# uiuc-robovision/video-dqn

Hardware: AMD Instinct MI355X
Metric: (s,a,r,s') TD-updates/sec, 224x224 frames, batch 256, 1/2/4/8 MI355X (higher is better)
Workload: dtype bf16; 1 GPU; HabitatDQNMultiAction ResNet-18 extra_capacity, 5 categories x 3 actions, full TD update (online fwd on [s;s'], target fwd on s', Double-DQN target + L2 TD loss, backward, Adam); batch_per_gpu=256, global_batch=256, frame=224x224x3 uint8 (normalise fused), parallelism=dp1, target_update_interval=1000, loss_clip=rect, loss_kind=l2, minibatch_pool=4, frame_pack=at the start of every update

## Files before the change

video_dqn_amd/csrc/engine.hip:

```cpp
#include "engine_net.h"

bool wgrad_two_stage() {
  static const bool on = [] { const char* e = getenv("VDQN_WGRAD_TWO_STAGE"); return e && e[0] == '1'; }();
  return on;
}

namespace {

bool side_ready(vdqn_net* net) {
  if (!net->overlap) return false;
  if (!net->side) {
    int prio = 0;
    {
      const char* e = getenv("VDQN_SIDE_PRIORITY");
      int lo = 0, hi = 0;
      if (hipDeviceGetStreamPriorityRange(&lo, &hi) == hipSuccess) prio = (!e || e[0] == 'l') ? lo : (e[0] == 'h' ? hi : 0);
    }
    if (hipStreamCreateWithPriority(&net->side, hipStreamNonBlocking, prio) != hipSuccess ||
        hipStreamCreateWithPriority(&net->side2, hipStreamNonBlocking, prio) != hipSuccess) {
      net->overlap = 0;
      net->side = nullptr;
      net->side2 = nullptr;
      return false;
    }
// ... 533 lines not shown
  }
  RC(run_dgrad(net, c1, pk, bw + W.g_h[b], gx, n, resid, x, st));
  return VDQN_OK;
}

}

extern "C" int vdqn_net_backward_begin(vdqn_net* net, const vdqn_step_args* a, const float* dq_f32, void* stream) {
  VDQN_CHECK(net && a && dq_f32, "vdqn_net_backward_begin: null arg");
  VDQN_CHECK(!net->basic(), "vdqn_net_backward_begin: only extra_capacity (eval-mode BatchNorm) has a per-call backward; ARCHITECTURE='basic' trains through vdqn_net_td_forward");
  VDQN_CHECK(a->params && a->bnstats && a->packed_online && a->acts_online && a->bwd && a->grads, "vdqn_net_backward_begin: null buffer");
  VDQN_CHECK(a->batch >= 1 && a->batch <= net->cfg.max_batch && a->acts_samples == a->batch,
             "vdqn_net_backward_begin: acts_samples (%d) must equal batch (%d) <= max_batch", a->acts_samples, a->batch);
  hipStream_t st = (hipStream_t)stream;
  const int B = a->batch;
  const BwdLayout W = bwd_layout(net, B);
  unsigned char* bw = (unsigned char*)a->bwd;
  hipError_t e = hipMemsetAsync(bw + W.zero_begin, 0, (size_t)W.zero_bytes, st);
  VDQN_CHECK(e == hipSuccess, "vdqn_net_backward_begin: memset failed: %s", hipGetErrorString(e));
  launch_dq_pad(net, dq_f32, bw + W.dq, B, st);
  VDQN_LAUNCH_CHECK();
  return VDQN_OK;
}

extern "C" void* vdqn_net_grad_stream(vdqn_net* net) {
  if (!net || !side_ready(net)) return nullptr;
  return (void*)net->side;
}

extern "C" int vdqn_net_backward_stage(vdqn_net* net, const vdqn_step_args* a, int32_t stage, void* stream) {
  VDQN_CHECK(net && a && a->grads, "vdqn_net_backward_stage: null arg");
  VDQN_CHECK(stage >= 0 && stage < 3, "vdqn_net_backward_stage: stage %d", stage);
  hipStream_t st = (hipStream_t)stream;
  const int B = a->batch, F = net->cfg.num_frames, n = B * F, dt = net->cfg.dtype;
  const bool gtb = a->train_on_ground_truth != 0;
  const ActLayout A = act_layout(net, step_layout_samples(net, a));
  const BwdLayout W = bwd_layout(net, B);
  const unsigned char* pk = (const unsigned char*)a->packed_online;
  unsigned char* ao = (unsigned char*)a->acts_online;
  unsigned char* bw = (unsigned char*)a->bwd;
  bool split_conv1 = false;
  int part_rows[kMaxLayers];
  std::fill(part_rows, part_rows + kMaxLayers, kTileRows);

  if (net->basic()) {
    if (stage == 0) {
      const Layer& top = net->layers[net->l_top4];
      RC(run_wgrad(net, top, bw, W, bw + W.dq, ao + A.avg, B, wgrad_stream(net, st), true));
      RC(run_dgrad(net, top, pk, bw + W.dq, bw + W.g_avg, B, nullptr, nullptr, st));
      RC(vdqn_avgpool_bwd(bw + W.g_avg, ao + A.o[7], bw + W.g_o[7], n, 49, 512, dt, st));
      RC(block_backward_train(net, a, 7, A, W, n, st));
      RC(block_backward_train(net, a, 6, A, W, n, st));
    } else if (stage == 1) {
      RC(block_backward_train(net, a, 5, A, W, n, st));
      RC(block_backward_train(net, a, 4, A, W, n, st));
    } else {
      for (int b = 3; b >= 0; --b) RC(block_backward_train(net, a, b, A, W, n, st));
      RC(vdqn_maxpool_bwd(bw + W.g_pool, ao + A.idx, nullptr, bw + W.g_c1, n, 112, 112, 64, dt, st));
      RC(run_bn_bwd(net, a, net->l_conv1, A, bw + W.g_c1, ao + A.r_c1, bw + W.g_c1, n, st));
      RC(run_wgrad(net, net->layers[net->l_conv1], bw, W, bw + W.g_c1, a->packed_frames ? a->packed_frames : ao + A.t_in, n, wgrad_stream(net, st)));
    }
  } else if (stage == 0) {
    const Layer& t4 = net->layers[net->l_top4];
    const Layer& t2 = net->layers[net->l_top2];
    const Layer& t0 = net->layers[net->l_top0];
    const Layer& f8 = net->layers[net->l_f8];
    RC(run_wgrad(net, t4, bw, W, bw + W.dq, ao + A.l1, B, wgrad_stream(net, st), true));
    RC(run_dgrad(net, t4, pk, bw + W.dq, bw + W.g_l1, B, nullptr, ao + A.l1, st, bw + W.part[kPartL1], nullptr, nullptr, &part_rows[net->l_top2]));
    RC(run_wgrad(net, t2, bw, W, bw + W.g_l1, ao + A.l0, B, wgrad_stream(net, st)));
    RC(run_dgrad(net, t2, pk, bw + W.g_l1, bw + W.g_l0, B, nullptr, ao + A.l0, st, bw + W.part[kPartL0], nullptr, nullptr, &part_rows[net->l_top0]));
    RC(run_wgrad(net, t0, bw, W, bw + W.g_l0, ao + A.f8, B, wgrad_stream(net, st)));
    RC(run_dgrad(net, t0, pk, bw + W.g_l0, bw + W.g_f8, B, nullptr, ao + A.f8, st, bw + W.part[kPartF8], nullptr, nullptr, &part_rows[net->l_f8]));
    RC(run_wgrad(net, f8, bw, W, bw + W.g_f8, ao + A.o[7], n, wgrad_stream(net, st)));
    RC(run_dgrad(net, f8, pk, bw + W.g_f8, bw + W.g_o[7], n, nullptr, ao + A.o[7], st, bw + W.part[part_o(7)]));
    RC(block_backward(net, a, 7, A, W, n, st));
    RC(block_backward(net, a, 6, A, W, n, st));
  } else if (stage == 1) {
    RC(block_backward(net, a, 5, A, W, n, st));
    RC(block_backward(net, a, 4, A, W, n, st));
  } else {
    for (int b = 3; b >= 0; --b) RC(block_backward(net, a, b, A, W, n, st));
    split_conv1 = net->overlap && net->side && net->l_conv1 == net->layer_stage_first[2] && net->layer_stage_count[2] > 1;
  }
  int max_co = 0;
  for (int i = net->layer_stage_first[stage]; i < net->layer_stage_first[stage] + net->layer_stage_count[stage]; ++i)
    max_co = net->layers[i].co > max_co ? net->layers[i].co : max_co;
  PartTable pt;
  memset(&pt, 0, sizeof(pt));
  for (int i = net->layer_stage_first[stage]; i < net->layer_stage_first[stage] + net->layer_stage_count[stage]; ++i) {
    const int buf = part_buf(net, i);
    if (buf < 0) continue;
    const PartInfo pi = part_info(net, buf, B, part_rows[i]);
    VDQN_CHECK(pi.entries <= pi.capacity, "vdqn_net_backward_stage: layer %s has %d column-sum entries, its buffer holds %lld",
               net->layers[i].name.c_str(), pi.entries, (long long)pi.capacity);
    pt.off[i] = W.part[buf]; pt.tiles[i] = pi.entries; pt.ld[i] = pi.ld; pt.groups[i] = pi.groups; pt.gstride[i] = pi.gstride;
  }
  const bool stem_tail = stage == 2 && !net->basic();
  auto conv1_chain = [&]() -> int {
    const Layer& L1 = net->layers[net->l_conv1];
    static const bool fuse_pool = [] { const char* e = getenv("VDQN_FUSE_POOL_BWD"); return !(e && e[0] == '0'); }();
    const int64_t det_need = net->cfg.deterministic ? vdqn_stem_wgrad_pool_workspace_bytes(n) : 0;
    if (fuse_pool && dt == VDQN_BF16 && (int64_t)n * 115 * 115 * 32 < (1ll << 31) && det_need <= W.det_ws_bytes) {
      prof_layer(L1, n);
      static const bool on_main_env = [] { const char* e = getenv("VDQN_STEM_WGRAD_MAIN"); return !(e && e[0] == '0'); }();
      const bool on_main = g_stem_wgrad_main_override >= 0 ? g_stem_wgrad_main_override != 0 : on_main_env;
      const bool main_st = on_main && split_conv1 && !net->cfg.deterministic;
      return vdqn_stem_wgrad_pool(bw + W.g_pool, ao + A.idx, a->packed_frames ? a->packed_frames : ao + A.t_in, reinterpret_cast<float*>(bw + L1.dw_off), n,
                                  net->cfg.deterministic ? bw + W.det_ws : nullptr, W.det_ws_bytes, main_st ? st : fork(net, st));
    }
    RC(vdqn_maxpool_bwd(bw + W.g_pool, ao + A.idx, nullptr, bw + W.g_c1, n, 112, 112, 64, dt, st));
    RC(run_wgrad(net, L1, bw, W, bw + W.g_c1, a->packed_frames ? a->packed_frames : ao + A.t_in, n, wgrad_stream(net, st)));
    return VDQN_OK;
  };
  if (stem_tail && !split_conv1) RC(conv1_chain());
  hipStream_t us = fork(net, st);
  if (wgrad_two_streams(net)) join(net, net->side2, net->side);
  const double unfold_bytes = (double)(net->stage_end[stage] - net->stage_begin[stage]) * 12.0;
  const int first = net->layer_stage_first[stage], count = net->layer_stage_count[stage];
  if (split_conv1) {
    launch_unfold(net, pt, first + 1, count - 1, max_co, 0, a, us, unfold_bytes);
    RC(conv1_chain());
    if (wgrad_two_streams(net)) join(net, net->side2, net->side);
    (void)fork(net, st);
    launch_unfold(net, pt, net->l_conv1, 1, net->layers[net->l_conv1].co, 0, a, net->side, 0.0);
  } else {
    launch_unfold(net, pt, first, count, max_co, net->basic() ? 1 : 0, a, us, unfold_bytes);
  }
  if (stage == 2) join(net, net->side, st);
  VDQN_LAUNCH_CHECK();
  return VDQN_OK;
}
```

video_dqn_amd/csrc/engine_net.h:

```cpp
#pragma once
#include <math.h>
#include <stdarg.h>
#include <stdlib.h>

#include <algorithm>
#include <string>
#include <vector>

#include "common.h"

#pragma GCC visibility push(hidden)

constexpr int kMaxLayers = 24;
constexpr float kBnEps = 1e-5f;
constexpr float kBnMomentum = 0.1f;

enum LayerKind { K_CONV = 0, K_CONV1_S2D = 1, K_LINEAR = 2, K_LINEAR_PERM = 3 };

struct Layer {
  std::string name, bn_name;
  int kind;
  int co, ci, r, s, stride, pad;
  int has_bn, has_bias;
  int k_ci, k_r, k_s, pix_stride;
// ... 16 lines not shown
  int tile_begin;
};
struct FoldTable {
  int n, n_tiles;
  FoldDesc d[kMaxLayers];
};
struct PartTable {
  int64_t off[kMaxLayers];
  int tiles[kMaxLayers], ld[kMaxLayers], groups[kMaxLayers], gstride[kMaxLayers];
};

enum PartBuf { kPartL1 = 0, kPartL0, kPartF8, kPartPool, kPartBlocks, kPartBufs = kPartBlocks + 16 };
inline int part_o(int b) { return kPartBlocks + 2 * b; }
inline int part_h(int b) { return kPartBlocks + 2 * b + 1; }
constexpr int kTileRows = 128;
struct PartInfo {
  int entries, ld, groups, gstride;
  int64_t capacity;
};

struct ActLayout {
  int64_t t_in, c1, pool, idx;
  int64_t h[8], o[8], ds[8];
  int64_t f8, l0, l1, q, qf;
  int64_t avg, r_c1, r_h[8], r_o[8], r_ds[8], bnw[kMaxLayers], bnw_begin, bnw_bytes, bn_sync;
  int64_t bn_det = -1, bn_det_bytes = 0;
  int64_t total;
};
struct BwdLayout {
  int64_t zero_begin, zero_bytes;
  int64_t dq, g_l1, g_l0, g_f8, g_o[8], g_h[8], dsg[8], g_pool, g_c1;
  int64_t part[kPartBufs];
  int64_t g_avg, g_or[8], g_dsr[8];
  int64_t det_ws, det_ws_bytes;
  int64_t total;
};

inline int64_t align_up(int64_t v, int64_t a = 256) { return (v + a - 1) / a * a; }

#pragma GCC visibility pop

struct vdqn_net {
  vdqn_net_config cfg;
  int gemm_dtype;
  int esz;
  std::vector<Layer> layers;
  std::vector<vdqn_param_info> params;
  int64_t trainable_numel, params_numel, bnstats_numel, packed_bytes;
  int64_t stage_begin[3], stage_end[3];
  int layer_stage_first[3], layer_stage_count[3];
  int64_t dw_bytes;
  FoldTable fold;
  int l_conv1, l_f8, l_top0, l_top2, l_top4;
  bool basic() const { return cfg.extra_capacity == 0; }
  int l_b_conv1[8], l_b_conv2[8], l_b_ds[8];
  BnSync bn_sync = {nullptr, nullptr, nullptr, 1};
  int wgrad_rr = 0;
  int overlap = 1;
  hipStream_t side = nullptr;
  hipStream_t side2 = nullptr;
  std::vector<hipEvent_t> events;
  size_t ev_next = 0;
};

#pragma GCC visibility push(hidden)

#define RC(x)                     \
  do {                            \
    int rc_ = (x);                \
    if (rc_ != VDQN_OK) return rc_; \
  } while (0)

inline int64_t frame_bytes(const vdqn_net* net) { return (int64_t)115 * 115 * 16 * net->esz; }
inline int block_planes(int b) { return 64 << (b / 2); }
inline int block_side(int b) { return 56 >> (b / 2); }

ActLayout act_layout(const vdqn_net* net, int n_samples);
BwdLayout bwd_layout(const vdqn_net* net, int n_samples);
vdqn_wgrad_args wgrad_shape_args(const vdqn_net* net, const Layer& L, int n_units);
int64_t wgrad_max_imgs(const vdqn_net* net, const Layer& L);
int part_buf(const vdqn_net* net, int li);
PartInfo part_info(const vdqn_net* net, int buf, int n_samples, int rows_per_entry);
bool wgrad_two_stage();
void launch_unfold(const vdqn_net* net, const PartTable& pt, int first_layer, int n_layers, int max_co, int raw, const vdqn_step_args* a,
                   hipStream_t stream, double bytes);
void launch_dq_pad(const vdqn_net* net, const float* dq_f32, void* dst, int rows, hipStream_t stream);

#pragma GCC visibility pop
```

video_dqn_amd/csrc/fold.hip:

```cpp
#include "engine_net.h"

namespace {

__device__ __forceinline__ long fold_src_index(const FoldDesc& d, int co, int k) {
  if (d.kind == K_CONV1_S2D) {
    const int a = k >> 6, j = (k >> 4) & 3, ch = k & 15;
    if (ch >= 12) return -1;
    const int bh = ch / 6, bw = (ch / 3) & 1, c = ch % 3;
    const int r7 = 2 * a + bh - 1, s7 = 2 * j + bw - 1;
    if (r7 < 0 || s7 < 0) return -1;
    return ((long)(co * 3 + c) * 7 + r7) * 7 + s7;
  } else if (d.kind == K_LINEAR_PERM) {
    const int f = k / 1600, rem = k - f * 1600;
    const int hw = rem >> 6, c = rem & 63;
    return (long)co * d.ci + f * 1600 + c * 25 + hw;
  } else {
    const int tap = k / d.k_ci, c = k - tap * d.k_ci;
    const int kr = tap / d.k_s, ks = tap - kr * d.k_s;
    return (((long)co * d.ci + c) * d.r + kr) * d.s + ks;
  }
}

__device__ __forceinline__ float fold_scale(const FoldDesc& d, const float* params, const float* bnstats, int co, int raw) {
  if (!d.has_bn || raw) return 1.0f;
  return params[d.g_off + co] / sqrtf(bnstats[d.var_off + co] + kBnEps);
}

template <typename T>
__global__ __launch_bounds__(256) void fold_kernel(const FoldTable tab, const float* __restrict__ params, const float* __restrict__ bnstats,
                                                   unsigned char* __restrict__ packed, int with_dgrad, int raw, int first_layer) {
  const FoldDesc& d = tab.d[first_layer + blockIdx.y];
  const int which = blockIdx.z;
  if (d.tiled) return;
  if (which == 1 && (!with_dgrad || d.wd_off < 0)) return;
  const long stride = (long)gridDim.x * blockDim.x;
  if (which == 0) {
    T* wf = reinterpret_cast<T*>(packed + d.wf_off);
    float* bias = reinterpret_cast<float*>(packed + d.bias_off);
    float* scale = reinterpret_cast<float*>(packed + d.scale_off);
    const long total = (long)d.co_pad * d.kf;
    for (long i = (long)blockIdx.x * blockDim.x + threadIdx.x; i < total; i += stride) {
      const int row = (int)(i / d.kf), k = (int)(i - (long)row * d.kf);
      float v = 0.f;
      if (row < d.co) {
        const float sc = fold_scale(d, params, bnstats, row, raw);
        const long src = fold_src_index(d, row, k);
        if (src >= 0) v = params[d.w_off + src] * sc;
        if (k == 0) {
          scale[row] = sc;
          float b = 0.f;
          if (d.has_bn) b = raw ? 0.f : params[d.b_off + row] - bnstats[d.mean_off + row] * sc;
          else if (d.has_bias) b = params[d.b_off + row];
          bias[row] = b;
        }
      } else if (k == 0) {
        scale[row] = 0.f;
        bias[row] = 0.f;
      }
      wf[i] = from_f32<T>(v);
    }
  } else {
    T* wd = reinterpret_cast<T*>(packed + d.wd_off);
    const long total = (long)d.cd_rows * d.kd;
    for (long i = (long)blockIdx.x * blockDim.x + threadIdx.x; i < total; i += stride) {
      const int n = (int)(i / d.kd), kk = (int)(i - (long)n * d.kd);
      const int tap = kk / d.co_pad, co = kk - tap * d.co_pad;
      float v = 0.f;
      if (co < d.co) {
        const long src = fold_src_index(d, co, tap * d.k_ci + n);
        if (src >= 0) v = params[d.w_off + src] * fold_scale(d, params, bnstats, co, raw);
      }
      wd[i] = from_f32<T>(v);
    }
  }
}

#ifndef VDQN_FOLD_COT
#define VDQN_FOLD_COT 32
#endif
constexpr int kFoldCot = VDQN_FOLD_COT;

template <typename T, int TAPS>
__device__ __forceinline__ void fold_tile_body(const FoldDesc& d, const float* __restrict__ params, const float* __restrict__ bnstats,
                                               unsigned char* __restrict__ packed, int with_dgrad, int raw, float* sW, float* s_scale, int t, int cot_sub) {
  constexpr int COT = kFoldCot;
  constexpr int RUN = 64 * TAPS;
  constexpr int PITCH = RUN + 1;
  const int ci_tiles = d.ci / 64;
  const int cot = t / ci_tiles, cit = t - cot * ci_tiles;
  const int co0 = cot * 64 + cot_sub * COT, c0 = cit * 64;
  if (threadIdx.x < COT) {
    const int co = co0 + threadIdx.x;
    const float sc = co < d.co ? fold_scale(d, params, bnstats, co, raw) : 0.f;
    s_scale[threadIdx.x] = sc;
    if (cit == 0) {
      float b = 0.f;
      if (co < d.co) {
        if (d.has_bn) b = raw ? 0.f : params[d.b_off + co] - bnstats[d.mean_off + co] * sc;
        else if (d.has_bias) b = params[d.b_off + co];
      }
      reinterpret_cast<float*>(packed + d.bias_off)[co] = b;
      reinterpret_cast<float*>(packed + d.scale_off)[co] = sc;
    }
  }
  __syncthreads();
#pragma unroll 6
  for (int i = threadIdx.x; i < COT * RUN / 4; i += 256) {
    const int co_l = i / (RUN / 4), q = i - co_l * (RUN / 4);
    const int co = co0 + co_l;
    float4 v = make_float4(0.f, 0.f, 0.f, 0.f);
    if (co < d.co) v = *reinterpret_cast<const float4*>(params + d.w_off + ((long)co * d.ci + c0) * TAPS + 4 * q);
    const float sc = s_scale[co_l];
    float* dst = sW + co_l * PITCH + 4 * q;
    dst[0] = v.x * sc; dst[1] = v.y * sc; dst[2] = v.z * sc; dst[3] = v.w * sc;
  }
  __syncthreads();
  T* wf = reinterpret_cast<T*>(packed + d.wf_off);
  constexpr int V16 = (int)(8 * sizeof(T) / 16);
#pragma unroll 3
  for (int i = threadIdx.x; i < COT * TAPS * 8; i += 256) {
    const int co_l = i / (TAPS * 8), rem = i - co_l * (TAPS * 8);
    const int tap = rem >> 3, c_l = (rem & 7) * 8;
    const float* src = sW + co_l * PITCH + c_l * TAPS + tap;
    T o8[8];
#pragma unroll
    for (int e = 0; e < 8; ++e) o8[e] = from_f32<T>(src[e * TAPS]);
    T* dst = wf + (long)(co0 + co_l) * d.kf + tap * d.ci + c0 + c_l;
#pragma unroll
    for (int v = 0; v < V16; ++v) reinterpret_cast<uint4*>(dst)[v] = reinterpret_cast<const uint4*>(o8)[v];
  }
  if (with_dgrad && d.wd_off >= 0) {
    T* wd = reinterpret_cast<T*>(packed + d.wd_off);
#pragma unroll 3
    for (int i = threadIdx.x; i < 64 * TAPS * (COT / 8); i += 256) {
      const int co_l = (i % (COT / 8)) * 8, rem = i / (COT / 8);
      const int tap = rem % TAPS, c_l = rem / TAPS;
      const float* src = sW + co_l * PITCH + c_l * TAPS + tap;
      T o8[8];
#pragma unroll
      for (int e = 0; e < 8; ++e) o8[e] = from_f32<T>(src[e * PITCH]);
      T* dst = wd + (long)(c0 + c_l) * d.kd + tap * d.co_pad + co0 + co_l;
#pragma unroll
      for (int v = 0; v < V16; ++v) reinterpret_cast<uint4*>(dst)[v] = reinterpret_cast<const uint4*>(o8)[v];
    }
  }
}

template <typename T>
__global__ __launch_bounds__(256) void fold_tile_kernel(const FoldTable tab, const float* __restrict__ params, const float* __restrict__ bnstats,
                                                        unsigned char* __restrict__ packed, int with_dgrad, int raw, int tile_first) {
  extern __shared__ __attribute__((aligned(16))) unsigned char fold_smem[];
  float* sW = reinterpret_cast<float*>(fold_smem);
  __shared__ float s_scale[32];
  int li = 0;
  for (int i = 0; i < tab.n; ++i)
    if (tab.d[i].tiled && tile_first + (int)blockIdx.x >= tab.d[i].tile_begin) li = i;
  const FoldDesc& d = tab.d[li];
  const int t = tile_first + (int)blockIdx.x - d.tile_begin;
  if (d.r * d.s == 9) fold_tile_body<T, 9>(d, params, bnstats, packed, with_dgrad, raw, sW, s_scale, t, (int)blockIdx.y);
  else fold_tile_body<T, 1>(d, params, bnstats, packed, with_dgrad, raw, sW, s_scale, t, (int)blockIdx.y);
}

__global__ __launch_bounds__(256) void unfold_kernel(const FoldTable tab, const PartTable pt, int first_layer, const float* __restrict__ params,
                                                     const float* __restrict__ bnstats, const unsigned char* __restrict__ bwd,
                                                     float* __restrict__ grads, int raw) {
  const FoldDesc& d = tab.d[first_layer + blockIdx.y];
  const int co = blockIdx.x;
  if (co >= d.co) return;
  const float* dw = reinterpret_cast<const float*>(bwd + d.dw_off) + (long)co * d.kf;
  const float* db = reinterpret_cast<const float*>(bwd + d.db_off);
  const int li = first_layer + blockIdx.y;
  float dbsum = 0.f;
  if (pt.tiles[li] > 0) {
    const float* part = reinterpret_cast<const float*>(bwd + pt.off[li]);
    const int per_tile = pt.groups[li];
    const int total = pt.tiles[li] * per_tile;
    for (int i = threadIdx.x; i < total; i += 256) {
      const int t = i / per_tile, g = i - t * per_tile;
      dbsum += part[(long)t * pt.ld[li] + g * pt.gstride[li] + co];
    }
  }
  float rstd = 1.f, sc = 1.f;
  if (d.has_bn && !raw) {
    rstd = 1.0f / sqrtf(bnstats[d.var_off + co] + kBnEps);
    sc = params[d.g_off + co] * rstd;
  }
  float dot = 0.f;
  __shared__ __attribute__((aligned(16))) float s_row[4608];
  if (d.tiled && d.kf <= 4608) {
    const int taps = d.r * d.s;
    const long base = d.w_off + (long)co * d.kf;
    if ((((uintptr_t)dw | (uintptr_t)(params + base) | (uintptr_t)(grads + base)) & 15) == 0 && (d.kf & 3) == 0) {
      for (int k = threadIdx.x; k < d.kf / 4; k += 256) reinterpret_cast<float4*>(s_row)[k] = reinterpret_cast<const float4*>(dw)[k];
      __syncthreads();
      for (int i4 = threadIdx.x; i4 < d.kf / 4; i4 += 256) {
        float g[4];
        int c = (4 * i4) / taps, tap = 4 * i4 - c * taps;
#pragma unroll
        for (int e = 0; e < 4; ++e) {
          g[e] = s_row[tap * d.ci + c];
          if (++tap == taps) { tap = 0; ++c; }
        }
        const float4 w = reinterpret_cast<const float4*>(params + base)[i4];
        reinterpret_cast<float4*>(grads + base)[i4] = make_float4(g[0] * sc, g[1] * sc, g[2] * sc, g[3] * sc);
        dot += g[0] * w.x + g[1] * w.y + g[2] * w.z + g[3] * w.w;
      }
    } else {
      for (int k = threadIdx.x; k < d.kf; k += 256) s_row[k] = dw[k];
      __syncthreads();
      for (int i = threadIdx.x; i < d.kf; i += 256) {
        const int c = i / taps, tap = i - c * taps;
        const float g = s_row[tap * d.ci + c];
        grads[base + i] = g * sc;
        dot += g * params[base + i];
      }
    }
  } else {
    for (int k = threadIdx.x; k < d.kf; k += 256) {
      const long src = fold_src_index(d, co, k);
      if (src >= 0) {
        const float g = dw[k];
        grads[d.w_off + src] = g * sc;
        dot += g * params[d.w_off + src];
      }
    }
  }
  __shared__ float red[8];
#pragma unroll
  for (int o = 32; o > 0; o >>= 1) {
    dot += __shfl_down(dot, o, 64);
    dbsum += __shfl_down(dbsum, o, 64);
  }
  if ((threadIdx.x & 63) == 0) {
    red[threadIdx.x >> 6] = dot;
    red[4 + (threadIdx.x >> 6)] = dbsum;
  }
  __syncthreads();
  if (threadIdx.x == 0) {
    const float tot = red[0] + red[1] + red[2] + red[3];
    const float dbp = pt.tiles[li] > 0 ? (red[4] + red[5] + red[6] + red[7]) : db[co];
    if (d.has_bn) {
      if (!raw) {
        grads[d.g_off + co] = rstd * (tot - bnstats[d.mean_off + co] * dbp);
        grads[d.b_off + co] = dbp;
      }
    } else if (d.has_bias) {
      grads[d.b_off + co] = dbp;
    }
  }
}

}

template <typename T>
__global__ __launch_bounds__(256) void dq_pad_kernel(const float* __restrict__ src, T* __restrict__ dst, int rows, int nq) {
  const int i = blockIdx.x * 256 + threadIdx.x;
  if (i >= rows * 64) return;
  const int b = i >> 6, c = i & 63;
  dst[i] = from_f32<T>(c < nq ? src[(long)b * nq + c] : 0.f);
}

static int pack_weights_layers(vdqn_net* net, const float* params, const float* bnstats, void* packed, int32_t with_dgrad, int first_layer,
                               int n_layers, hipStream_t stream) {
  if (n_layers <= 0) return VDQN_OK;
  dim3 grid(256, (unsigned)n_layers, 2);
  const int dgrad = with_dgrad & 1, raw = (with_dgrad >> 1) & 1;
  int tile_first = -1, tile_end = 0;
  for (int i = first_layer; i < first_layer + n_layers; ++i) {
    const FoldDesc& d = net->fold.d[i];
    if (!d.tiled) continue;
    if (tile_first < 0) tile_first = d.tile_begin;
    tile_end = d.tile_begin + (d.co_pad / 64) * (d.ci / 64);
  }
  const double share = (double)n_layers / (double)net->layers.size();
  ProfScope ps_("fold_weights", 0.0, ((double)net->trainable_numel * 4.0 + (double)net->packed_bytes * (dgrad ? 1.0 : 0.5)) * share, stream);
  const size_t tile_smem = kFoldCot * (64 * 9 + 1) * 4;
  vdqn_ensure_dyn_smem(reinterpret_cast<const void*>(&fold_tile_kernel<bf16raw>), (size_t)tile_smem);
  vdqn_ensure_dyn_smem(reinterpret_cast<const void*>(&fold_tile_kernel<float>), (size_t)tile_smem);
  if (net->cfg.dtype == VDQN_BF16) {
    hipLaunchKernelGGL((fold_kernel<bf16raw>), grid, dim3(256), 0, stream, net->fold, params, bnstats, (unsigned char*)packed, dgrad, raw, first_layer);
    if (tile_first >= 0)
      hipLaunchKernelGGL((fold_tile_kernel<bf16raw>), dim3(tile_end - tile_first, 64 / kFoldCot), dim3(256), tile_smem, stream, net->fold, params, bnstats,
                         (unsigned char*)packed, dgrad, raw, tile_first);
  } else {
    hipLaunchKernelGGL((fold_kernel<float>), grid, dim3(256), 0, stream, net->fold, params, bnstats, (unsigned char*)packed, dgrad, raw, first_layer);
    if (tile_first >= 0)
      hipLaunchKernelGGL((fold_tile_kernel<float>), dim3(tile_end - tile_first, 64 / kFoldCot), dim3(256), tile_smem, stream, net->fold, params, bnstats,
                         (unsigned char*)packed, dgrad, raw, tile_first);
  }
  VDQN_LAUNCH_CHECK();
  return VDQN_OK;
}

extern "C" int vdqn_net_pack_weights(vdqn_net* net, const float* params, const float* bnstats, void* packed, int32_t with_dgrad, void* stream) {
  VDQN_CHECK(net && params && bnstats && packed, "vdqn_net_pack_weights: null arg");
  return pack_weights_layers(net, params, bnstats, packed, with_dgrad, 0, (int)net->layers.size(), (hipStream_t)stream);
}

void launch_dq_pad(const vdqn_net* net, const float* dq_f32, void* dst, int rows, hipStream_t stream) {
  const int nq = net->cfg.action_dim * net->cfg.num_classes;
  const int blocks = (rows * 64 + 255) / 256;
  if (net->cfg.dtype == VDQN_BF16)
    hipLaunchKernelGGL((dq_pad_kernel<bf16raw>), dim3(blocks), dim3(256), 0, stream, dq_f32, reinterpret_cast<bf16raw*>(dst), rows, nq);
  else
    hipLaunchKernelGGL((dq_pad_kernel<float>), dim3(blocks), dim3(256), 0, stream, dq_f32, reinterpret_cast<float*>(dst), rows, nq);
}

void launch_unfold(const vdqn_net* net, const PartTable& pt, int first_layer, int n_layers, int max_co, int raw, const vdqn_step_args* a,
                   hipStream_t stream, double bytes) {
  ProfScope ps_("unfold_grads", 0.0, bytes, stream);
  hipLaunchKernelGGL(unfold_kernel, dim3(max_co, n_layers), dim3(256), 0, stream, net->fold, pt, first_layer, a->params, a->bnstats,
                     (const unsigned char*)a->bwd, a->grads, raw);
}
```

Before: 42660 tuples/s.

## Rework weight fold and grad unfold kernels into flattened per-layer work lists

Weight folding becomes a single launch over a flattened list of work items. Each layer gets a tiled transpose mode (3x3, 1x1, or a permuted linear mode with 25 taps) or chunked elementwise work, and blocks are ordered by stage. This replaces the separate elementwise and tile launches, shrinks tiles, and stages bf16 in LDS to cut LDS footprint. Gradient unfolding likewise replaces the max_co-by-layers grid, with its many idle blocks, by a compact work list where each wave handles several output rows with vectorized loads. The cost is more complex indexing and alignment checks that fall back to per-row blocks.

Measured after the change: 40600 tuples/s. 4.8% lower.

```diff
diff --git a/video_dqn_amd/csrc/engine.hip b/video_dqn_amd/csrc/engine.hip
--- a/video_dqn_amd/csrc/engine.hip
+++ b/video_dqn_amd/csrc/engine.hip
@@ -639,9 +639,6 @@
     for (int b = 3; b >= 0; --b) RC(block_backward(net, a, b, A, W, n, st));
     split_conv1 = net->overlap && net->side && net->l_conv1 == net->layer_stage_first[2] && net->layer_stage_count[2] > 1;
   }
-  int max_co = 0;
-  for (int i = net->layer_stage_first[stage]; i < net->layer_stage_first[stage] + net->layer_stage_count[stage]; ++i)
-    max_co = net->layers[i].co > max_co ? net->layers[i].co : max_co;
   PartTable pt;
   memset(&pt, 0, sizeof(pt));
   for (int i = net->layer_stage_first[stage]; i < net->layer_stage_first[stage] + net->layer_stage_count[stage]; ++i) {
@@ -675,13 +672,13 @@
   const double unfold_bytes = (double)(net->stage_end[stage] - net->stage_begin[stage]) * 12.0;
   const int first = net->layer_stage_first[stage], count = net->layer_stage_count[stage];
   if (split_conv1) {
-    launch_unfold(net, pt, first + 1, count - 1, max_co, 0, a, us, unfold_bytes);
+    launch_unfold(net, pt, first + 1, count - 1, 0, a, us, unfold_bytes);
     RC(conv1_chain());
     if (wgrad_two_streams(net)) join(net, net->side2, net->side);
     (void)fork(net, st);
-    launch_unfold(net, pt, net->l_conv1, 1, net->layers[net->l_conv1].co, 0, a, net->side, 0.0);
+    launch_unfold(net, pt, net->l_conv1, 1, 0, a, net->side, 0.0);
   } else {
-    launch_unfold(net, pt, first, count, max_co, net->basic() ? 1 : 0, a, us, unfold_bytes);
+    launch_unfold(net, pt, first, count, net->basic() ? 1 : 0, a, us, unfold_bytes);
   }
   if (stage == 2) join(net, net->side, st);
   VDQN_LAUNCH_CHECK();
diff --git a/video_dqn_amd/csrc/engine_net.h b/video_dqn_amd/csrc/engine_net.h
--- a/video_dqn_amd/csrc/engine_net.h
+++ b/video_dqn_amd/csrc/engine_net.h
@@ -122,7 +122,7 @@
 int part_buf(const vdqn_net* net, int li);
 PartInfo part_info(const vdqn_net* net, int buf, int n_samples, int rows_per_entry);
 bool wgrad_two_stage();
-void launch_unfold(const vdqn_net* net, const PartTable& pt, int first_layer, int n_layers, int max_co, int raw, const vdqn_step_args* a,
+void launch_unfold(const vdqn_net* net, const PartTable& pt, int first_layer, int n_layers, int raw, const vdqn_step_args* a,
                    hipStream_t stream, double bytes);
 void launch_dq_pad(const vdqn_net* net, const float* dq_f32, void* dst, int rows, hipStream_t stream);
 
diff --git a/video_dqn_amd/csrc/fold.hip b/video_dqn_amd/csrc/fold.hip
--- a/video_dqn_amd/csrc/fold.hip
+++ b/video_dqn_amd/csrc/fold.hip
@@ -26,20 +26,175 @@
   return params[d.g_off + co] / sqrtf(bnstats[d.var_off + co] + kBnEps);
 }
 
+enum FoldMode { kFoldElem = 0, kFoldTile1 = 1, kFoldTile9 = 2, kFoldPerm = 3 };
+constexpr int kFoldElemChunk = 2048;
+struct FoldWork {
+  int n;
+  int begin[kMaxLayers + 1];
+  int layer[kMaxLayers];
+  int mode[kMaxLayers];
+};
+
+inline int fold_mode(const FoldDesc& d) {
+  const bool lin64 = (d.kind == K_CONV || d.kind == K_LINEAR) && d.ci % 64 == 0 && d.co_pad % 64 == 0 && d.k_ci == d.ci;
+  if (lin64 && d.r * d.s == 9 && d.k_s == 3) return kFoldTile9;
+  if (lin64 && d.r * d.s == 1) return kFoldTile1;
+  if (d.kind == K_LINEAR_PERM && d.ci % 1600 == 0 && d.k_ci == d.ci && d.kf == d.ci && d.kd == d.co_pad && d.co_pad % 64 == 0) return kFoldPerm;
+  return kFoldElem;
+}
+
+template <int TAPS> struct FoldTileShape;
+template <> struct FoldTileShape<9> { static constexpr int CT = 32, COT = 32; };
+template <> struct FoldTileShape<1> { static constexpr int CT = 64, COT = 32; };
+template <> struct FoldTileShape<25> { static constexpr int CT = 32, COT = 16; };
+template <typename T> constexpr int fold_pitch(int run) { return sizeof(T) == 2 ? run + 2 : run + 1; }
+template <typename T, int TAPS> constexpr size_t fold_tile_smem() {
+  return (size_t)FoldTileShape<TAPS>::COT * fold_pitch<T>(FoldTileShape<TAPS>::CT * TAPS) * sizeof(T);
+}
+
+inline int fold_blocks(const FoldDesc& d, int mode, int dgrad) {
+  switch (mode) {
+    case kFoldTile9: return (d.co_pad / FoldTileShape<9>::COT) * (d.ci / FoldTileShape<9>::CT);
+    case kFoldTile1: return (d.co_pad / FoldTileShape<1>::COT) * (d.ci / FoldTileShape<1>::CT);
+    case kFoldPerm: return (d.co_pad / FoldTileShape<25>::COT) * (d.ci / 1600) * (64 / FoldTileShape<25>::CT);
+    default: {
+      const long nf = ((long)d.co_pad * d.kf + kFoldElemChunk - 1) / kFoldElemChunk;
+      const long nd = (dgrad && d.wd_off >= 0) ? ((long)d.cd_rows * d.kd + kFoldElemChunk - 1) / kFoldElemChunk : 0;
+      return (int)(nf + nd);
+    }
+  }
+}
+
+__device__ __forceinline__ void fold_lds_store4(float* dst, float a, float b, float c, float e) {
+  dst[0] = a; dst[1] = b; dst[2] = c; dst[3] = e;
+}
+__device__ __forceinline__ void fold_lds_store4(bf16raw* dst, float a, float b, float c, float e) {
+  uint32_t* p = reinterpret_cast<uint32_t*>(dst);
+  p[0] = (uint32_t)from_f32<bf16raw>(a) | ((uint32_t)from_f32<bf16raw>(b) << 16);
+  p[1] = (uint32_t)from_f32<bf16raw>(c) | ((uint32_t)from_f32<bf16raw>(e) << 16);
+}
+
+template <typename T, int TAPS, bool PERM>
+__device__ __forceinline__ void fold_tile_body(const FoldDesc& d, const float* __restrict__ params, const float* __restrict__ bnstats,
+                                               unsigned char* __restrict__ packed, int with_dgrad, int raw, T* sW, float* s_scale, int t) {
+  constexpr int CT = FoldTileShape<TAPS>::CT, COT = FoldTileShape<TAPS>::COT;
+  constexpr int RUN = CT * TAPS;
+  constexpr int PITCH = fold_pitch<T>(RUN);
+  constexpr int Q = RUN / 4, NQ = COT * Q, NLD = (NQ + 255) / 256;
+  const int tid = threadIdx.x;
+  int co0, src_pitch, wf_tap;
+  long src_col0, wf_col0, wd_row0, wd_tap;
+  bool first_col;
+  if (PERM) {
+    constexpr int HALVES = 64 / CT;
+    const int per_cot = (d.ci / 1600) * HALVES;
+    const int cot = t / per_cot, rem = t - cot * per_cot;
+    const int f = rem / HALVES, c0 = (rem - f * HALVES) * CT;
+    co0 = cot * COT;
+    src_pitch = d.ci;
+    src_col0 = (long)f * 1600 + c0 * TAPS;
+    wf_col0 = (long)f * 1600 + c0; wf_tap = 64;
+    wd_row0 = (long)f * 1600 + c0; wd_tap = (long)64 * d.kd;
+    first_col = rem == 0;
+  } else {
+    const int ci_tiles = d.ci / CT;
+    const int cot = t / ci_tiles, cit = t - cot * ci_tiles;
+    const int c0 = cit * CT;
+    co0 = cot * COT;
+    src_pitch = d.ci * TAPS;
+    src_col0 = (long)c0 * TAPS;
+    wf_col0 = c0; wf_tap = d.ci;
+    wd_row0 = c0; wd_tap = d.co_pad;
+    first_col = cit == 0;
+  }
+  const float* src = params + d.w_off + (long)co0 * src_pitch + src_col0;
+  float4 v[NLD];
+#pragma unroll
+  for (int j = 0; j < NLD; ++j) {
+    const int i = tid + 256 * j;
+    v[j] = make_float4(0.f, 0.f, 0.f, 0.f);
+    if (NQ % 256 == 0 || i < NQ) {
+      const int co_l = i / Q, q = i - co_l * Q;
+      if (co0 + co_l < d.co) v[j] = *reinterpret_cast<const float4*>(src + (long)co_l * src_pitch + 4 * q);
+    }
+  }
+  if (tid < COT) {
+    const int co = co0 + tid;
+    const float sc = co < d.co ? fold_scale(d, params, bnstats, co, raw) : 0.f;
+    s_scale[tid] = sc;
+    if (first_col) {
+      float b = 0.f;
+      if (co < d.co) {
+        if (d.has_bn) b = raw ? 0.f : params[d.b_off + co] - bnstats[d.mean_off + co] * sc;
+        else if (d.has_bias) b = params[d.b_off + co];
+      }
+      reinterpret_cast<float*>(packed + d.bias_off)[co] = b;
+      reinterpret_cast<float*>(packed + d.scale_off)[co] = sc;
+    }
+  }
+  __syncthreads();
+#pragma unroll
+  for (int j = 0; j < NLD; ++j) {
+    const int i = tid + 256 * j;
+    if (NQ % 256 == 0 || i < NQ) {
+      const int co_l = i / Q, q = i - co_l * Q;
+      const float sc = s_scale[co_l];
+      fold_lds_store4(sW + co_l * PITCH + 4 * q, v[j].x * sc, v[j].y * sc, v[j].z * sc, v[j].w * sc);
+    }
+  }
+  __syncthreads();
+  constexpr int V16 = (int)(8 * sizeof(T) / 16);
+  {
+    T* wf = reinterpret_cast<T*>(packed + d.wf_off) + (long)co0 * d.kf + wf_col0;
+    constexpr int CG = CT / 8, N = COT * TAPS * CG;
+#pragma unroll
+    for (int j = 0; j < (N + 255) / 256; ++j) {
+      const int i = tid + 256 * j;
+      if (N % 256 == 0 || i < N) {
+        const int co_l = i / (TAPS * CG), rem = i - co_l * (TAPS * CG);
+        const int tap = rem / CG, c_l = (rem - tap * CG) * 8;
+        const T* s = sW + co_l * PITCH + c_l * TAPS + tap;
+        alignas(16) T o8[8];
+#pragma unroll
+        for (int e = 0; e < 8; ++e) o8[e] = s[e * TAPS];
+        T* dst = wf + (long)co_l * d.kf + (long)tap * wf_tap + c_l;
+#pragma unroll
+        for (int u = 0; u < V16; ++u) reinterpret_cast<uint4*>(dst)[u] = reinterpret_cast<const uint4*>(o8)[u];
+      }
+    }
+  }
+  if (with_dgrad && d.wd_off >= 0) {
+    T* wd = reinterpret_cast<T*>(packed + d.wd_off) + wd_row0 * d.kd + co0;
+    constexpr int OG = COT / 8, N = CT * TAPS * OG;
+#pragma unroll
+    for (int j = 0; j < (N + 255) / 256; ++j) {
+      const int i = tid + 256 * j;
+      if (N % 256 == 0 || i < N) {
+        const int rem = i / OG, co_l = (i - rem * OG) * 8;
+        const int c_l = rem / TAPS, tap = rem - c_l * TAPS;
+        const T* s = sW + co_l * PITCH + c_l * TAPS + tap;
+        alignas(16) T o8[8];
+#pragma unroll
+        for (int e = 0; e < 8; ++e) o8[e] = s[e * PITCH];
+        T* dst = wd + (long)c_l * d.kd + (long)tap * wd_tap + co_l;
+#pragma unroll
+        for (int u = 0; u < V16; ++u) reinterpret_cast<uint4*>(dst)[u] = reinterpret_cast<const uint4*>(o8)[u];
+      }
+    }
+  }
+}
+
 template <typename T>
-__global__ __launch_bounds__(256) void fold_kernel(const FoldTable tab, const float* __restrict__ params, const float* __restrict__ bnstats,
-                                                   unsigned char* __restrict__ packed, int with_dgrad, int raw, int first_layer) {
-  const FoldDesc& d = tab.d[first_layer + blockIdx.y];
-  const int which = blockIdx.z;
-  if (d.tiled) return;
-  if (which == 1 && (!with_dgrad || d.wd_off < 0)) return;
-  const long stride = (long)gridDim.x * blockDim.x;
-  if (which == 0) {
+__device__ __forceinline__ void fold_elem_body(const FoldDesc& d, const float* __restrict__ params, const float* __restrict__ bnstats,
+                                               unsigned char* __restrict__ packed, int raw, int t) {
+  const long total_f = (long)d.co_pad * d.kf;
+  const int nf = (int)((total_f + kFoldElemChunk - 1) / kFoldElemChunk);
+  if (t < nf) {
     T* wf = reinterpret_cast<T*>(packed + d.wf_off);
     float* bias = reinterpret_cast<float*>(packed + d.bias_off);
     float* scale = reinterpret_cast<float*>(packed + d.scale_off);
-    const long total = (long)d.co_pad * d.kf;
-    for (long i = (long)blockIdx.x * blockDim.x + threadIdx.x; i < total; i += stride) {
+    const long end = min(total_f, (long)(t + 1) * kFoldElemChunk);
+    for (long i = (long)t * kFoldElemChunk + threadIdx.x; i < end; i += 256) {
       const int row = (int)(i / d.kf), k = (int)(i - (long)row * d.kf);
       float v = 0.f;
       if (row < d.co) {
@@ -61,8 +216,9 @@
     }
   } else {
     T* wd = reinterpret_cast<T*>(packed + d.wd_off);
-    const long total = (long)d.cd_rows * d.kd;
-    for (long i = (long)blockIdx.x * blockDim.x + threadIdx.x; i < total; i += stride) {
+    const long total_d = (long)d.cd_rows * d.kd;
+    const long end = min(total_d, (long)(t - nf + 1) * kFoldElemChunk);
+    for (long i = (long)(t - nf) * kFoldElemChunk + threadIdx.x; i < end; i += 256) {
       const int n = (int)(i / d.kd), kk = (int)(i - (long)n * d.kd);
       const int tap = kk / d.co_pad, co = kk - tap * d.co_pad;
       float v = 0.f;
@@ -75,109 +231,88 @@
   }
 }
 
-#ifndef VDQN_FOLD_COT
-#define VDQN_FOLD_COT 32
-#endif
-constexpr int kFoldCot = VDQN_FOLD_COT;
-
-template <typename T, int TAPS>
-__device__ __forceinline__ void fold_tile_body(const FoldDesc& d, const float* __restrict__ params, const float* __restrict__ bnstats,
-                                               unsigned char* __restrict__ packed, int with_dgrad, int raw, float* sW, float* s_scale, int t, int cot_sub) {
-  constexpr int COT = kFoldCot;
-  constexpr int RUN = 64 * TAPS;
-  constexpr int PITCH = RUN + 1;
-  const int ci_tiles = d.ci / 64;
-  const int cot = t / ci_tiles, cit = t - cot * ci_tiles;
-  const int co0 = cot * 64 + cot_sub * COT, c0 = cit * 64;
-  if (threadIdx.x < COT) {
-    const int co = co0 + threadIdx.x;
-    const float sc = co < d.co ? fold_scale(d, params, bnstats, co, raw) : 0.f;
-    s_scale[threadIdx.x] = sc;
-    if (cit == 0) {
-      float b = 0.f;
-      if (co < d.co) {
-        if (d.has_bn) b = raw ? 0.f : params[d.b_off + co] - bnstats[d.mean_off + co] * sc;
-        else if (d.has_bias) b = params[d.b_off + co];
-      }
-      reinterpret_cast<float*>(packed + d.bias_off)[co] = b;
-      reinterpret_cast<float*>(packed + d.scale_off)[co] = sc;
-    }
-  }
-  __syncthreads();
-#pragma unroll 6
-  for (int i = threadIdx.x; i < COT * RUN / 4; i += 256) {
-    const int co_l = i / (RUN / 4), q = i - co_l * (RUN / 4);
-    const int co = co0 + co_l;
-    float4 v = make_float4(0.f, 0.f, 0.f, 0.f);
-    if (co < d.co) v = *reinterpret_cast<const float4*>(params + d.w_off + ((long)co * d.ci + c0) * TAPS + 4 * q);
-    const float sc = s_scale[co_l];
-    float* dst = sW + co_l * PITCH + 4 * q;
-    dst[0] = v.x * sc; dst[1] = v.y * sc; dst[2] = v.z * sc; dst[3] = v.w * sc;
-  }
-  __syncthreads();
-  T* wf = reinterpret_cast<T*>(packed + d.wf_off);
-  constexpr int V16 = (int)(8 * sizeof(T) / 16);
-#pragma unroll 3
-  for (int i = threadIdx.x; i < COT * TAPS * 8; i += 256) {
-    const int co_l = i / (TAPS * 8), rem = i - co_l * (TAPS * 8);
-    const int tap = rem >> 3, c_l = (rem & 7) * 8;
-    const float* src = sW + co_l * PITCH + c_l * TAPS + tap;
-    T o8[8];
-#pragma unroll
-    for (int e = 0; e < 8; ++e) o8[e] = from_f32<T>(src[e * TAPS]);
-    T* dst = wf + (long)(co0 + co_l) * d.kf + tap * d.ci + c0 + c_l;
-#pragma unroll
-    for (int v = 0; v < V16; ++v) reinterpret_cast<uint4*>(dst)[v] = reinterpret_cast<const uint4*>(o8)[v];
-  }
-  if (with_dgrad && d.wd_off >= 0) {
-    T* wd = reinterpret_cast<T*>(packed + d.wd_off);
-#pragma unroll 3
-    for (int i = threadIdx.x; i < 64 * TAPS * (COT / 8); i += 256) {
-      const int co_l = (i % (COT / 8)) * 8, rem = i / (COT / 8);
-      const int tap = rem % TAPS, c_l = rem / TAPS;
-      const float* src = sW + co_l * PITCH + c_l * TAPS + tap;
-      T o8[8];
-#pragma unroll
-      for (int e = 0; e < 8; ++e) o8[e] = from_f32<T>(src[e * PITCH]);
-      T* dst = wd + (long)(c0 + c_l) * d.kd + tap * d.co_pad + co0 + co_l;
-#pragma unroll
-      for (int v = 0; v < V16; ++v) reinterpret_cast<uint4*>(dst)[v] = reinterpret_cast<const uint4*>(o8)[v];
-    }
-  }
-}
-
 template <typename T>
-__global__ __launch_bounds__(256) void fold_tile_kernel(const FoldTable tab, const float* __restrict__ params, const float* __restrict__ bnstats,
-                                                        unsigned char* __restrict__ packed, int with_dgrad, int raw, int tile_first) {
+__global__ __launch_bounds__(256) void fold_kernel(const FoldTable tab, const FoldWork work, const float* __restrict__ params,
+                                                   const float* __restrict__ bnstats, unsigned char* __restrict__ packed, int with_dgrad, int raw) {
   extern __shared__ __attribute__((aligned(16))) unsigned char fold_smem[];
-  float* sW = reinterpret_cast<float*>(fold_smem);
+  T* sW = reinterpret_cast<T*>(fold_smem);
   __shared__ float s_scale[32];
-  int li = 0;
-  for (int i = 0; i < tab.n; ++i)
-    if (tab.d[i].tiled && tile_first + (int)blockIdx.x >= tab.d[i].tile_begin) li = i;
-  const FoldDesc& d = tab.d[li];
-  const int t = tile_first + (int)blockIdx.x - d.tile_begin;
-  if (d.r * d.s == 9) fold_tile_body<T, 9>(d, params, bnstats, packed, with_dgrad, raw, sW, s_scale, t, (int)blockIdx.y);
-  else fold_tile_body<T, 1>(d, params, bnstats, packed, with_dgrad, raw, sW, s_scale, t, (int)blockIdx.y);
-}
-
-__global__ __launch_bounds__(256) void unfold_kernel(const FoldTable tab, const PartTable pt, int first_layer, const float* __restrict__ params,
-                                                     const float* __restrict__ bnstats, const unsigned char* __restrict__ bwd,
-                                                     float* __restrict__ grads, int raw) {
-  const FoldDesc& d = tab.d[first_layer + blockIdx.y];
-  const int co = blockIdx.x;
-  if (co >= d.co) return;
+  int e = 0;
+  for (int i = 1; i < work.n; ++i)
+    if ((int)blockIdx.x >= work.begin[i]) e = i;
+  const FoldDesc& d = tab.d[work.layer[e]];
+  const int t = (int)blockIdx.x - work.begin[e];
+  switch (work.mode[e]) {
+    case kFoldTile9: fold_tile_body<T, 9, false>(d, params, bnstats, packed, with_dgrad, raw, sW, s_scale, t); break;
+    case kFoldTile1: fold_tile_body<T, 1, false>(d, params, bnstats, packed, with_dgrad, raw, sW, s_scale, t); break;
+    case kFoldPerm: fold_tile_body<T, 25, true>(d, params, bnstats, packed, with_dgrad, raw, sW, s_scale, t); break;
+    default: fold_elem_body<T>(d, params, bnstats, packed, raw, t); break;
+  }
+}
+
+struct UnfoldWork {
+  int n;
+  int begin[kMaxLayers + 1];
+  int layer[kMaxLayers];
+  int rpw[kMaxLayers];
+};
+constexpr int kUnfoldRow = 4608;
+constexpr int kUnfoldWaveRow = 1152;
+
+__device__ __forceinline__ void unfold_gather4(const float* s_row, int i4, int taps, int ci, float g[4]) {
+  int c = (4 * i4) / taps, tap = 4 * i4 - c * taps;
+#pragma unroll
+  for (int e = 0; e < 4; ++e) {
+    g[e] = s_row[tap * ci + c];
+    if (++tap == taps) { tap = 0; ++c; }
+  }
+}
+
+__device__ __forceinline__ long unfold_part_index(int i, int per_tile, int ld, int gstride) {
+  if (per_tile == 1) return (long)i * ld;
+  const int t = i / per_tile, g = i - t * per_tile;
+  return (long)t * ld + g * gstride;
+}
+
+__device__ __forceinline__ void unfold_row_block(const FoldDesc& d, const PartTable& pt, int li, int co, const float* __restrict__ params,
+                                                 const float* __restrict__ bnstats, const unsigned char* __restrict__ bwd,
+                                                 float* __restrict__ grads, int raw, float* s_row, float* red) {
   const float* dw = reinterpret_cast<const float*>(bwd + d.dw_off) + (long)co * d.kf;
   const float* db = reinterpret_cast<const float*>(bwd + d.db_off);
-  const int li = first_layer + blockIdx.y;
+  const bool row_lds = d.tiled && d.kf <= kUnfoldRow;
+  const long base = d.w_off + (long)co * d.kf;
+  const bool vec = row_lds && (((uintptr_t)dw | (uintptr_t)(params + base) | (uintptr_t)(grads + base)) & 15) == 0 && (d.kf & 3) == 0;
+  constexpr int NV = kUnfoldRow / 4 / 256 + 1;
+  float4 dwv[NV], wv[NV];
+#pragma unroll
+  for (int j = 0; j < NV; ++j) dwv[j] = wv[j] = make_float4(0.f, 0.f, 0.f, 0.f);
+  if (vec) {
+#pragma unroll
+    for (int j = 0; j < NV; ++j) {
+      const int i4 = threadIdx.x + 256 * j;
+      dwv[j] = wv[j] = make_float4(0.f, 0.f, 0.f, 0.f);
+      if (i4 < d.kf / 4) {
+        dwv[j] = reinterpret_cast<const float4*>(dw)[i4];
+        wv[j] = reinterpret_cast<const float4*>(params + base)[i4];
+      }
+    }
+  }
   float dbsum = 0.f;
   if (pt.tiles[li] > 0) {
-    const float* part = reinterpret_cast<const float*>(bwd + pt.off[li]);
-    const int per_tile = pt.groups[li];
+    const float* part = reinterpret_cast<const float*>(bwd + pt.off[li]) + co;
+    const int per_tile = pt.groups[li], ld = pt.ld[li], gstride = pt.gstride[li];
     const int total = pt.tiles[li] * per_tile;
-    for (int i = threadIdx.x; i < total; i += 256) {
-      const int t = i / per_tile, g = i - t * per_tile;
-      dbsum += part[(long)t * pt.ld[li] + g * pt.gstride[li] + co];
+    for (int i0 = threadIdx.x; i0 < total; i0 += 256 * 16) {
+      float p[16];
+#pragma unroll
+      for (int u = 0; u < 16; ++u) {
+        const int i = i0 + 256 * u;
+        p[u] = 0.f;
+        if (i < total) p[u] = part[unfold_part_index(i, per_tile, ld, gstride)];
+      }
+#pragma unroll
+      for (int u = 0; u < 16; ++u)
+        if (i0 + 256 * u < total) dbsum += p[u];
     }
   }
   float rstd = 1.f, sc = 1.f;
@@ -186,24 +321,25 @@
     sc = params[d.g_off + co] * rstd;
   }
   float dot = 0.f;
-  __shared__ __attribute__((aligned(16))) float s_row[4608];
-  if (d.tiled && d.kf <= 4608) {
+  if (row_lds) {
     const int taps = d.r * d.s;
-    const long base = d.w_off + (long)co * d.kf;
-    if ((((uintptr_t)dw | (uintptr_t)(params + base) | (uintptr_t)(grads + base)) & 15) == 0 && (d.kf & 3) == 0) {
-      for (int k = threadIdx.x; k < d.kf / 4; k += 256) reinterpret_cast<float4*>(s_row)[k] = reinterpret_cast<const float4*>(dw)[k];
+    if (vec) {
+#pragma unroll
+      for (int j = 0; j < NV; ++j) {
+        const int i4 = threadIdx.x + 256 * j;
+        if (i4 < d.kf / 4) reinterpret_cast<float4*>(s_row)[i4] = dwv[j];
+      }
       __syncthreads();
-      for (int i4 = threadIdx.x; i4 < d.kf / 4; i4 += 256) {
-        float g[4];
-        int c = (4 * i4) / taps, tap = 4 * i4 - c * taps;
-#pragma unroll
-        for (int e = 0; e < 4; ++e) {
-          g[e] = s_row[tap * d.ci + c];
-          if (++tap == taps) { tap = 0; ++c; }
+#pragma unroll
+      for (int j = 0; j < NV; ++j) {
+        const int i4 = threadIdx.x + 256 * j;
+        if (i4 < d.kf / 4) {
+          float g[4];
+          unfold_gather4(s_row, i4, taps, d.ci, g);
+          const float4 w = wv[j];
+          reinterpret_cast<float4*>(grads + base)[i4] = make_float4(g[0] * sc, g[1] * sc, g[2] * sc, g[3] * sc);
+          dot += g[0] * w.x + g[1] * w.y + g[2] * w.z + g[3] * w.w;
         }
-        const float4 w = reinterpret_cast<const float4*>(params + base)[i4];
-        reinterpret_cast<float4*>(grads + base)[i4] = make_float4(g[0] * sc, g[1] * sc, g[2] * sc, g[3] * sc);
-        dot += g[0] * w.x + g[1] * w.y + g[2] * w.z + g[3] * w.w;
       }
     } else {
       for (int k = threadIdx.x; k < d.kf; k += 256) s_row[k] = dw[k];
@@ -225,7 +361,6 @@
       }
     }
   }
-  __shared__ float red[8];
 #pragma unroll
   for (int o = 32; o > 0; o >>= 1) {
     dot += __shfl_down(dot, o, 64);
@@ -250,6 +385,147 @@
   }
 }
 
+template <int RPW>
+__device__ __forceinline__ void unfold_rows_wave(const FoldDesc& d, const PartTable& pt, int li, int t, const float* __restrict__ params,
+                                                 const float* __restrict__ bnstats, const unsigned char* __restrict__ bwd,
+                                                 float* __restrict__ grads, int raw, float* s_row, float* red) {
+  constexpr int R = 4 * RPW;
+  constexpr int NV = kUnfoldWaveRow / 4 / 64 + 1;
+  constexpr int NJ = (kUnfoldWaveRow / 4 / RPW + 63) / 64;
+  constexpr int PB = 64 / R;
+  const int tid = threadIdx.x, wave = tid >> 6, lane = tid & 63;
+  const int co0 = t * R, co_w = co0 + wave * RPW;
+  const int kf = d.kf, q4 = kf >> 2, n4 = RPW * q4, taps = d.r * d.s;
+  const bool parts = pt.tiles[li] > 0;
+  float dbs[R];
+#pragma unroll
+  for (int r = 0; r < R; ++r) dbs[r] = 0.f;
+  if (parts) {
+    const float* part = reinterpret_cast<const float*>(bwd + pt.off[li]) + co0;
+    const int per_tile = pt.groups[li], ld = pt.ld[li], gstride = pt.gstride[li];
+    const int total = pt.tiles[li] * per_tile;
+    for (int i0 = tid; i0 < total; i0 += 256 * PB) {
+      float4 x[PB][R / 4];
+#pragma unroll
+      for (int u = 0; u < PB; ++u) {
+        const int i = i0 + 256 * u;
+#pragma unroll
+        for (int v = 0; v < R / 4; ++v) x[u][v] = make_float4(0.f, 0.f, 0.f, 0.f);
+        if (i < total) {
+          const float4* p = reinterpret_cast<const float4*>(part + unfold_part_index(i, per_tile, ld, gstride));
+#pragma unroll
+          for (int v = 0; v < R / 4; ++v) x[u][v] = p[v];
+        }
+      }
+#pragma unroll
+      for (int u = 0; u < PB; ++u) {
+        if (i0 + 256 * u < total) {
+#pragma unroll
+          for (int v = 0; v < R / 4; ++v) {
+            dbs[4 * v + 0] += x[u][v].x; dbs[4 * v + 1] += x[u][v].y; dbs[4 * v + 2] += x[u][v].z; dbs[4 * v + 3] += x[u][v].w;
+          }
+        }
+      }
+    }
+  }
+  const float4* dw4 = reinterpret_cast<const float4*>(reinterpret_cast<const float*>(bwd + d.dw_off) + (long)co_w * kf);
+  float4 dwv[NV];
+#pragma unroll
+  for (int j = 0; j < NV; ++j) {
+    const int i = lane + 64 * j;
+    dwv[j] = make_float4(0.f, 0.f, 0.f, 0.f);
+    if (i < n4) dwv[j] = dw4[i];
+  }
+  float4 wv[RPW][NJ];
+#pragma unroll
+  for (int r = 0; r < RPW; ++r) {
+    const float4* w4 = reinterpret_cast<const float4*>(params + d.w_off + (long)(co_w + r) * kf);
+#pragma unroll
+    for (int j = 0; j < NJ; ++j) {
+      const int i4 = lane + 64 * j;
+      wv[r][j] = make_float4(0.f, 0.f, 0.f, 0.f);
+      if (i4 < q4) wv[r][j] = w4[i4];
+    }
+  }
+  float* s_w = s_row + wave * kUnfoldWaveRow;
+#pragma unroll
+  for (int j = 0; j < NV; ++j) {
+    const int i = lane + 64 * j;
+    if (i < n4) reinterpret_cast<float4*>(s_w)[i] = dwv[j];
+  }
+#pragma unroll
+  for (int r = 0; r < R; ++r) {
+#pragma unroll
+    for (int o = 32; o > 0; o >>= 1) dbs[r] += __shfl_down(dbs[r], o, 64);
+  }
+  if (lane == 0) {
+#pragma unroll
+    for (int r = 0; r < R; ++r) red[r * 4 + wave] = dbs[r];
+  }
+  __syncthreads();
+  const float* db = reinterpret_cast<const float*>(bwd + d.db_off);
+#pragma unroll
+  for (int r = 0; r < RPW; ++r) {
+    const int co = co_w + r;
+    float rstd = 1.f, sc = 1.f;
+    if (d.has_bn && !raw) {
+      rstd = 1.0f / sqrtf(bnstats[d.var_off + co] + kBnEps);
+      sc = params[d.g_off + co] * rstd;
+    }
+    const float* s_r = s_w + r * kf;
+    float4* g4 = reinterpret_cast<float4*>(grads + d.w_off + (long)co * kf);
+    float acc[4] = {0.f, 0.f, 0.f, 0.f};
+#pragma unroll
+    for (int j = 0; j < NJ; ++j) {
+      const int i4 = lane + 64 * j;
+      if (i4 < q4) {
+        float g[4];
+        unfold_gather4(s_r, i4, taps, d.ci, g);
+        const float4 w = wv[r][j];
+        g4[i4] = make_float4(g[0] * sc, g[1] * sc, g[2] * sc, g[3] * sc);
+        acc[j & 3] += g[0] * w.x + g[1] * w.y + g[2] * w.z + g[3] * w.w;
+      }
+    }
+#pragma unroll
+    for (int q = 0; q < 4; ++q) {
+#pragma unroll
+      for (int o = 32; o > 0; o >>= 1) acc[q] += __shfl_down(acc[q], o, 64);
+    }
+    if (lane == 0) {
+      const float tot = acc[0] + acc[1] + acc[2] + acc[3];
+      const float* rd = red + (wave * RPW + r) * 4;
+      const float dbp = parts ? (rd[0] + rd[1] + rd[2] + rd[3]) : db[co];
+      if (d.has_bn) {
+        if (!raw) {
+          grads[d.g_off + co] = rstd * (tot - bnstats[d.mean_off + co] * dbp);
+          grads[d.b_off + co] = dbp;
+        }
+      } else if (d.has_bias) {
+        grads[d.b_off + co] = dbp;
+      }
+    }
+  }
+}
+
+__global__ __launch_bounds__(256) void unfold_kernel(const FoldTable tab, const PartTable pt, const UnfoldWork work, const float* __restrict__ params,
+                                                     const float* __restrict__ bnstats, const unsigned char* __restrict__ bwd,
+                                                     float* __restrict__ grads, int raw) {
+  __shared__ __attribute__((aligned(16))) float s_row[kUnfoldRow];
+  __shared__ float red[64];
+  int e = 0;
+  for (int i = 1; i < work.n; ++i)
+    if ((int)blockIdx.x >= work.begin[i]) e = i;
+  const int li = work.layer[e];
+  const FoldDesc& d = tab.d[li];
+  const int t = (int)blockIdx.x - work.begin[e];
+  switch (work.rpw[e]) {
+    case 1: unfold_rows_wave<1>(d, pt, li, t, params, bnstats, bwd, grads, raw, s_row, red); break;
+    case 2: unfold_rows_wave<2>(d, pt, li, t, params, bnstats, bwd, grads, raw, s_row, red); break;
+    case 4: unfold_rows_wave<4>(d, pt, li, t, params, bnstats, bwd, grads, raw, s_row, red); break;
+    default: unfold_row_block(d, pt, li, t, params, bnstats, bwd, grads, raw, s_row, red); break;
+  }
+}
+
 }
 
 template <typename T>
@@ -263,30 +539,37 @@
 static int pack_weights_layers(vdqn_net* net, const float* params, const float* bnstats, void* packed, int32_t with_dgrad, int first_layer,
                                int n_layers, hipStream_t stream) {
   if (n_layers <= 0) return VDQN_OK;
-  dim3 grid(256, (unsigned)n_layers, 2);
   const int dgrad = with_dgrad & 1, raw = (with_dgrad >> 1) & 1;
-  int tile_first = -1, tile_end = 0;
-  for (int i = first_layer; i < first_layer + n_layers; ++i) {
-    const FoldDesc& d = net->fold.d[i];
-    if (!d.tiled) continue;
-    if (tile_first < 0) tile_first = d.tile_begin;
-    tile_end = d.tile_begin + (d.co_pad / 64) * (d.ci / 64);
-  }
+  const bool bf16 = net->cfg.dtype == VDQN_BF16;
+  FoldWork work;
+  memset(&work, 0, sizeof(work));
+  size_t smem = 0;
+  for (int st = 2; st >= 0; --st) {
+    for (int i = first_layer; i < first_layer + n_layers; ++i) {
+      if (net->layers[i].stage != st) continue;
+      const FoldDesc& d = net->fold.d[i];
+      const int mode = fold_mode(d);
+      size_t need = 0;
+      if (mode == kFoldTile9) need = bf16 ? fold_tile_smem<bf16raw, 9>() : fold_tile_smem<float, 9>();
+      else if (mode == kFoldTile1) need = bf16 ? fold_tile_smem<bf16raw, 1>() : fold_tile_smem<float, 1>();
+      else if (mode == kFoldPerm) need = bf16 ? fold_tile_smem<bf16raw, 25>() : fold_tile_smem<float, 25>();
+      smem = need > smem ? need : smem;
+      const int e = work.n++;
+      work.layer[e] = i;
+      work.mode[e] = mode;
+      work.begin[e + 1] = work.begin[e] + fold_blocks(d, mode, dgrad);
+    }
+  }
+  VDQN_CHECK(work.n == n_layers, "pack_weights_layers: %d of %d layers have a stage", work.n, n_layers);
   const double share = (double)n_layers / (double)net->layers.size();
   ProfScope ps_("fold_weights", 0.0, ((double)net->trainable_numel * 4.0 + (double)net->packed_bytes * (dgrad ? 1.0 : 0.5)) * share, stream);
-  const size_t tile_smem = kFoldCot * (64 * 9 + 1) * 4;
-  vdqn_ensure_dyn_smem(reinterpret_cast<const void*>(&fold_tile_kernel<bf16raw>), (size_t)tile_smem);
-  vdqn_ensure_dyn_smem(reinterpret_cast<const void*>(&fold_tile_kernel<float>), (size_t)tile_smem);
-  if (net->cfg.dtype == VDQN_BF16) {
-    hipLaunchKernelGGL((fold_kernel<bf16raw>), grid, dim3(256), 0, stream, net->fold, params, bnstats, (unsigned char*)packed, dgrad, raw, first_layer);
-    if (tile_first >= 0)
-      hipLaunchKernelGGL((fold_tile_kernel<bf16raw>), dim3(tile_end - tile_first, 64 / kFoldCot), dim3(256), tile_smem, stream, net->fold, params, bnstats,
-                         (unsigned char*)packed, dgrad, raw, tile_first);
+  const dim3 grid((unsigned)work.begin[work.n]);
+  if (bf16) {
+    vdqn_ensure_dyn_smem(reinterpret_cast<const void*>(&fold_kernel<bf16raw>), smem);
+    hipLaunchKernelGGL((fold_kernel<bf16raw>), grid, dim3(256), smem, stream, net->fold, work, params, bnstats, (unsigned char*)packed, dgrad, raw);
   } else {
-    hipLaunchKernelGGL((fold_kernel<float>), grid, dim3(256), 0, stream, net->fold, params, bnstats, (unsigned char*)packed, dgrad, raw, first_layer);
-    if (tile_first >= 0)
-      hipLaunchKernelGGL((fold_tile_kernel<float>), dim3(tile_end - tile_first, 64 / kFoldCot), dim3(256), tile_smem, stream, net->fold, params, bnstats,
-                         (unsigned char*)packed, dgrad, raw, tile_first);
+    vdqn_ensure_dyn_smem(reinterpret_cast<const void*>(&fold_kernel<float>), smem);
+    hipLaunchKernelGGL((fold_kernel<float>), grid, dim3(256), smem, stream, net->fold, work, params, bnstats, (unsigned char*)packed, dgrad, raw);
   }
   VDQN_LAUNCH_CHECK();
   return VDQN_OK;
@@ -306,9 +589,27 @@
     hipLaunchKernelGGL((dq_pad_kernel<float>), dim3(blocks), dim3(256), 0, stream, dq_f32, reinterpret_cast<float*>(dst), rows, nq);
 }
 
-void launch_unfold(const vdqn_net* net, const PartTable& pt, int first_layer, int n_layers, int max_co, int raw, const vdqn_step_args* a,
+void launch_unfold(const vdqn_net* net, const PartTable& pt, int first_layer, int n_layers, int raw, const vdqn_step_args* a,
                    hipStream_t stream, double bytes) {
+  if (n_layers <= 0) return;
   ProfScope ps_("unfold_grads", 0.0, bytes, stream);
-  hipLaunchKernelGGL(unfold_kernel, dim3(max_co, n_layers), dim3(256), 0, stream, net->fold, pt, first_layer, a->params, a->bnstats,
+  const bool aligned = (((uintptr_t)a->params | (uintptr_t)a->grads | (uintptr_t)a->bwd) & 15) == 0;
+  UnfoldWork work;
+  memset(&work, 0, sizeof(work));
+  for (int i = first_layer; i < first_layer + n_layers; ++i) {
+    const FoldDesc& d = net->fold.d[i];
+    int rpw = 0;
+    if (aligned && d.tiled && d.kf <= kUnfoldWaveRow && d.kf % 4 == 0 && d.w_off % 4 == 0 && d.dw_off % 16 == 0) {
+      rpw = kUnfoldWaveRow / d.kf >= 4 ? 4 : kUnfoldWaveRow / d.kf;
+      if (rpw == 3) rpw = 2;
+      if (d.co % (4 * rpw) != 0) rpw = 0;
+      if (rpw && pt.tiles[i] > 0 && (pt.off[i] % 16 != 0 || pt.ld[i] % 4 != 0 || pt.gstride[i] % 4 != 0)) rpw = 0;
+    }
+    const int e = work.n++;
+    work.layer[e] = i;
+    work.rpw[e] = rpw;
+    work.begin[e + 1] = work.begin[e] + (rpw ? d.co / (4 * rpw) : d.co);
+  }
+  hipLaunchKernelGGL(unfold_kernel, dim3((unsigned)work.begin[work.n]), dim3(256), 0, stream, net->fold, pt, work, a->params, a->bnstats,
                      (const unsigned char*)a->bwd, a->grads, raw);
 }
```
